# casselineau/Tracer

Measured on AMD Instinct MI355X. Metric: Mray-bounces/s on Sandia NSTTF field, higher is better.
Workload: dtype f64

## Files before the change

### tracer_amd/csrc/trc_bounds.h

```cpp
#ifndef TRC_BOUNDS_H
#define TRC_BOUNDS_H

#include <cmath>
#include <cstdlib>
#include <cstring>
#include <limits>
#include <vector>
#include "trc_core.h"

static inline bool trc_surface_local_box(const trc_surface_desc &s, double l[3], double h[3], bool *global_axes) {
    const double *g = s.gm;
    *global_axes = false;
    switch (s.gm_kind) {
    case TRC_GM_RECT: case TRC_GM_RECT_EXTRUDED: case TRC_GM_RECT_PERFORATED:
        l[0] = -g[0]; h[0] = g[0]; l[1] = -g[1]; h[1] = g[1]; l[2] = h[2] = 0.0; break;
    case TRC_GM_ROUND: case TRC_GM_ROUND_CUT:
        l[0] = l[1] = -g[0]; h[0] = h[1] = g[0]; l[2] = h[2] = 0.0; break;
    case TRC_GM_TRIANGLE:
        for (int i = 0; i < 3; ++i) { l[i] = std::fmin(0.0, std::fmin(g[i], g[3 + i])); h[i] = std::fmax(0.0, std::fmax(g[i], g[3 + i])); }
        break;
    case TRC_GM_POLYGON:
        l[0] = g[2]; h[0] = g[3]; l[1] = g[4]; h[1] = g[5]; l[2] = h[2] = 0.0; break;
    case TRC_GM_PARAB_DISH: {
        double rx = std::sqrt(g[2] / g[0]), ry = std::sqrt(g[2] / g[1]);
        l[0] = -rx; h[0] = rx; l[1] = -ry; h[1] = ry; l[2] = 0.0; h[2] = g[2]; break;
// ... 195 lines not shown
}

struct trc_accel_host {
    std::vector<float> sbox;
    std::vector<float> obb;
    std::vector<int32_t> unbounded;
    std::vector<uint32_t> nodes;
    std::vector<uint16_t> leaf_surfs;
    std::vector<uint16_t> brute_leaf;
    uint32_t brute_nodes[2];
    float brute_root[6];
    float root[6];
    float delta;
    double cen[3], slo[3], shi[3];
    bool any_bounded;
    int kd_depth;
    bool grid_ok;
    int32_t grid_dim[3];
    float grid_lo[3], grid_cs[3], grid_inv[3];
    std::vector<uint16_t> grid_off;
    std::vector<uint16_t> grid_list;
    std::vector<int32_t> grid_apart;
    float grid_root[6];
    bool big_ok;
    std::vector<int32_t> big_apart;
    int32_t big_dim[3];
    float big_lo[3], big_cs[3], big_inv[3], big_root[6];
    std::vector<uint32_t> big_off, big_list;
    std::vector<float> big_ent;
    std::vector<uint32_t> big_occ;
};

static inline void trc_accel_build_surfaces(const trc_surface_desc *surfs, int n, trc_accel_host &A) {
    const double INF = std::numeric_limits<double>::infinity();
    std::vector<double> lo(3 * (size_t)n), hi(3 * (size_t)n);
    std::vector<char> bounded(n);
    double slo[3] = {INF, INF, INF}, shi[3] = {-INF, -INF, -INF};
    A.unbounded.clear();
    A.any_bounded = false;
    for (int i = 0; i < n; ++i) {
        bounded[i] = trc_surface_bounds(surfs[i], &lo[3 * (size_t)i], &hi[3 * (size_t)i]);
        if (bounded[i]) {
            A.any_bounded = true;
            for (int k = 0; k < 3; ++k) { slo[k] = std::fmin(slo[k], lo[3 * (size_t)i + k]); shi[k] = std::fmax(shi[k], hi[3 * (size_t)i + k]); }
        } else A.unbounded.push_back(i);
    }
// ... 136 lines not shown
                range[6 * j + k] = a; range[6 * j + 3 + k] = z;
                c *= (size_t)(z - a + 1);
            }
            total += c;
        }
        if (total > 65535) continue;
        for (size_t j = 0; j < nb; ++j)
            for (int z = range[6 * j + 2]; z <= range[6 * j + 5]; ++z)
                for (int y = range[6 * j + 1]; y <= range[6 * j + 4]; ++y)
                    for (int x = range[6 * j]; x <= range[6 * j + 3]; ++x) count[((size_t)z * dim[1] + y) * dim[0] + x + 1]++;
        for (size_t c = 0; c < cells; ++c) count[c + 1] += count[c];
        A.grid_off.assign(cells + 1, 0);
        for (size_t c = 0; c <= cells; ++c) A.grid_off[c] = (uint16_t)count[c];
        A.grid_list.assign(total > 0 ? total : 1, 0);
        std::vector<uint32_t> cur(count.begin(), count.end() - 1);
        for (size_t j = 0; j < nb; ++j)
            for (int z = range[6 * j + 2]; z <= range[6 * j + 5]; ++z)
                for (int y = range[6 * j + 1]; y <= range[6 * j + 4]; ++y)
                    for (int x = range[6 * j]; x <= range[6 * j + 3]; ++x)
                        A.grid_list[cur[((size_t)z * dim[1] + y) * dim[0] + x]++] = members[j];
        for (int k = 0; k < 3; ++k) { A.grid_dim[k] = dim[k]; A.grid_lo[k] = (float)lo[k]; A.grid_cs[k] = cs[k]; A.grid_inv[k] = inv[k]; }
        A.grid_ok = true;
        return;
    }
}

static inline bool trc_tri_box_overlap(const double c[3], const double h[3], const double v0[3], const double v1[3], const double v2[3]) {
    double a[3][3], e[3][3];
    for (int i = 0; i < 3; ++i) { a[0][i] = v0[i] - c[i]; a[1][i] = v1[i] - c[i]; a[2][i] = v2[i] - c[i]; }
    for (int i = 0; i < 3; ++i) { e[0][i] = a[1][i] - a[0][i]; e[1][i] = a[2][i] - a[1][i]; e[2][i] = a[0][i] - a[2][i]; }
    double scale = 0.0;
    for (int k = 0; k < 3; ++k) for (int i = 0; i < 3; ++i) scale = std::fmax(scale, std::fabs(a[k][i]));
    for (int i = 0; i < 3; ++i) scale = std::fmax(scale, h[i]);
    const double tol = 1e-12 * scale;
    for (int i = 0; i < 3; ++i) {
        const double mn = std::fmin(a[0][i], std::fmin(a[1][i], a[2][i])), mx = std::fmax(a[0][i], std::fmax(a[1][i], a[2][i]));
        if (mn > h[i] + tol || mx < -h[i] - tol) return false;
    }
    {
        const double n[3] = {e[0][1] * e[1][2] - e[0][2] * e[1][1], e[0][2] * e[1][0] - e[0][0] * e[1][2], e[0][0] * e[1][1] - e[0][1] * e[1][0]};
        const double d = n[0] * a[0][0] + n[1] * a[0][1] + n[2] * a[0][2];
        const double rr = h[0] * std::fabs(n[0]) + h[1] * std::fabs(n[1]) + h[2] * std::fabs(n[2]);
        if (std::fabs(d) > rr + tol * (std::fabs(n[0]) + std::fabs(n[1]) + std::fabs(n[2]))) return false;
    }
    for (int k = 0; k < 3; ++k)
        for (int i = 0; i < 3; ++i) {
// ... 247 lines not shown
```

### tracer_amd/csrc/trc_core.h

```cpp
#ifndef TRC_CORE_H
#define TRC_CORE_H

#include <stdint.h>
#include <math.h>
#include "../../include/tracer_amd.h"

#if defined(__HIPCC__)
#define TRC_HD __host__ __device__ __forceinline__
#define TRC_HD_NOINLINE __host__ __device__
#else
#define TRC_HD static inline
#define TRC_HD_NOINLINE static
#endif

#define TRC_INF (__builtin_inf())
#define TRC_INF32 (__builtin_inff())
#define TRC_NAN (__builtin_nan(""))
#define TRC_TWO_PI 6.283185307179586476925286766559
#define TRC_PI 3.14159265358979323846264338327950288
#define TRC_BUIE_TABLE (3 * (TRC_BUIE_NELEM + 1) + 6)
#define TRC_BUIE_STAGED (TRC_BUIE_TABLE + 3)

#define TRC_REC_HDR 14

// ... 585 lines not shown
    float ax = (b[0] - r.ox) * r.ix, bx = (b[3] - r.ox) * r.ix;
    float ay = (b[1] - r.oy) * r.iy, by = (b[4] - r.oy) * r.iy;
    float az = (b[2] - r.oz) * r.iz, bz = (b[5] - r.oz) * r.iz;
    float lo = fmaxf(fmaxf(fminf(ax, bx), fminf(ay, by)), fmaxf(fminf(az, bz), 0.0f));
    float hi = fminf(fminf(fmaxf(ax, bx), fmaxf(ay, by)), fmaxf(az, bz));
    return hi * 1.0001f + 1e-6f >= lo;
}

TRC_HD bool trc_obb_hit32(const float *B, float ox, float oy, float oz, float dx, float dy, float dz) {
    const float rx = ox - B[3], ry = oy - B[7], rz = oz - B[11];
    const float lx = B[0] * rx + B[1] * ry + B[2] * rz, ly = B[4] * rx + B[5] * ry + B[6] * rz, lz = B[8] * rx + B[9] * ry + B[10] * rz;
    const float ex = B[0] * dx + B[1] * dy + B[2] * dz, ey = B[4] * dx + B[5] * dy + B[6] * dz, ez = B[8] * dx + B[9] * dy + B[10] * dz;
#if defined(__HIP_DEVICE_COMPILE__)
    const float ix = __builtin_amdgcn_rcpf(ex), iy = __builtin_amdgcn_rcpf(ey), iz = __builtin_amdgcn_rcpf(ez);
#else
    const float ix = 1.0f / ex, iy = 1.0f / ey, iz = 1.0f / ez;
#endif
    const float ax = (B[12] - lx) * ix, bx = (B[15] - lx) * ix;
    const float ay = (B[13] - ly) * iy, by = (B[16] - ly) * iy;
    const float az = (B[14] - lz) * iz, bz = (B[17] - lz) * iz;
    const float lo = fmaxf(fmaxf(fminf(ax, bx), fminf(ay, by)), fmaxf(fminf(az, bz), 0.0f));
    const float hi = fminf(fminf(fmaxf(ax, bx), fmaxf(ay, by)), fmaxf(az, bz));
    return hi * 1.0001f + 1e-6f >= lo;
}

TRC_HD bool trc_tri_hit32(float v0x, float v0y, float v0z, float e1x, float e1y, float e1z, float E, float e2x, float e2y, float e2z,
                          float emax2, float delta, const trc_ray32 &r) {
    const float tx = r.ox - v0x, ty = r.oy - v0y, tz = r.oz - v0z;
    const float px = fmaf(r.dy, e2z, -(r.dz * e2y)), py = fmaf(r.dz, e2x, -(r.dx * e2z)), pz = fmaf(r.dx, e2y, -(r.dy * e2x));
    const float det = fmaf(e1x, px, fmaf(e1y, py, e1z * pz));
    const float qx = fmaf(ty, e1z, -(tz * e1y)), qy = fmaf(tz, e1x, -(tx * e1z)), qz = fmaf(tx, e1y, -(ty * e1x));
    float u = fmaf(tx, px, fmaf(ty, py, tz * pz));
    float v = fmaf(r.dx, qx, fmaf(r.dy, qy, r.dz * qz));
    float tn = fmaf(e2x, qx, fmaf(e2y, qy, e2z * qz));
    if (det < 0.0f) { u = -u; v = -v; tn = -tn; }
    const float ad = fabsf(det);
    if (!(ad > 1e-5f * emax2)) return true;
    return u >= -E && v >= -E && u + v <= ad + 2.0f * E && tn >= -delta * (ad + emax2);
}

TRC_HD uint32_t trc_kd32_step(uint32_t w0, uint32_t w1, const trc_ray32 &r, float delta, float tmin, float *tmax,
                              bool *push, uint32_t *push_na, float *push_t) {
    uint32_t axis = w1 & 3u;
    float split = __builtin_bit_cast(float, w0);
    float o = axis == 0 ? r.ox : (axis == 1 ? r.oy : r.oz);
    float iv = axis == 0 ? r.ix : (axis == 1 ? r.iy : r.iz);
// ... 1418 lines not shown
```

### tracer_amd/csrc/trc_device.h

```cpp
#ifndef TRC_DEVICE_H
#define TRC_DEVICE_H

#include <hip/hip_runtime.h>
#include "trc_core.h"
#include "trc_bounds.h"
#include "trc_footprint.h"
#include "trc_forms.h"

struct FluxMapDev {
    int32_t surf, nu, nv, chart;
    int64_t edges_u, edges_v;
    int64_t bins;
    double proj[12];
};
static_assert(sizeof(FluxMapDev) == 136, "tests/shade_cases.py (SIZEOF_FLUXMAPDEV) restates this size in the sums of the LDS images");

struct DScene {
    const double *recs;
    const double *opt;
    const int32_t *sflags;
    const double *extra;
    int32_t stride, n_surf, n_extra, has_kd;
    const int32_t *kd_a, *kd_b, *kd_leaf, *kd_always;
    const double *kd_split;
// ... 399 lines not shown
    int static_general;
    FpDev fp;
    int static_first;
    int lds_recs;
    int lds_tables;
    int lds_fm_bins;
    int lds_extra;
    int bounce_no;
    int bg_occ_words;
    int split_terminal;
    unsigned chunk_thit;
    int search;
    int shade_cls;
    int shade_term_cls;
    long long act_base0;
    unsigned chunk_hitbuf;
    const uint32_t *hl_slot, *hl_surf;
    const double *hl_t;
    long long hl_room;
    int hl_cn;
    unsigned part_chunk[3];
    int part_static[3];
    CarryIn carry;
};

template <class ARGS>
__device__ __forceinline__ const ARGS *kernel_args_again() {
    static_assert(std::is_trivially_copyable<ARGS>::value, "the block is read as the bytes the launch copied into the segment");
    auto p = __builtin_amdgcn_kernarg_segment_ptr();
    asm volatile("" : "+s"(p));
    return (const ARGS *)p;
}

#define TRC_SURF_CLS_SHIFT 17
#define TRC_SURF_CLS_MASK 0x3
template <int THREADS>
__device__ __forceinline__ int wg_next(int i) {
    if constexpr (THREADS > 0) return i + THREADS;
    else return i + blockDim.x;
}

__device__ __forceinline__ void nearest_linked(const SCand *q3n, uint32_t k, double &t, int &s) {
    while (k != SQ_INVALID) {
        const SCand c = q3n[k];
        if (c.t < t || (c.t == t && (int)c.surf < s)) { t = c.t; s = (int)c.surf; }
        k = c.next;
// ... 255 lines not shown
```

### tracer_amd/csrc/trc_forms.h

```cpp
#ifndef TRC_FORMS_H
#define TRC_FORMS_H

#include <cstdio>
#include "trc_bounds.h"
#include "trc_footprint.h"

#define SC_THREADS 512
#define SC_GEN_CAP 1024
#define SF_THREADS(FLAT) ((FLAT) ? 1024 : 768)
#define SF2_DERIVES_CELL(FLAT, LDS) ((FLAT) || (LDS))
#ifndef SW_LEAFCAP
#define SW_LEAFCAP 16
#endif
#ifndef SW_LIST_T
#define SW_LIST_T uint16_t
#endif
#ifndef SW_THREADS
#define SW_THREADS 256
#endif
#define SB_THREADS 1024
#define SB_THREADS_OF(GRIDM) (SB_THREADS)
#define SA_THREADS 1024
#ifndef SHC_THREADS
#define SHC_THREADS 1024
// ... 76 lines not shown
    p.tables = p.sbox = lds;
    p.flags = flags;
    if (grid_cells) { p.grid_cells = grid_cells; p.grid_list = grid_list; }
    p.coop_waves = coop_waves;
    return p;
}
static inline size_t lds_need(const trc_lds_layout &L) { return L.end + L.slack; }
static inline size_t lds_request(const trc_lds_layout &L) { return lds_need(L) + 16; }
static inline size_t shade_lds_need(const trc_shade_parts &p) { const trc_shade_layout L = trc_shade_lds_layout(p); return L.end + L.slack; }

struct StreamKnobs {
    int search;
    bool fresh;
    bool bounce;
    bool first;
    bool coop;
    int absorb;
    bool static_chunks;
    bool room_set; long long room;
    long long q3_entries;
    int fp_cells;
    bool umask;
    int slots;
};

struct trc_scene_facts {
    int n_surf, stride;
    bool accel_ok, accel_kd_ok, has_kd;
    int kd_nodes, kd_nleaf, kd_nalways, kd_depth;
    bool grid_ok, big_ok;
    int grid_cells, grid_list;
    int brute_list, n_unbounded;
    int big_occ_words;
    int n_fm_edges, fms_bytes, n_extra;
    long long fm_bins;
    bool chart;
    bool transfer;
    bool splits;
    bool walked;
    bool all_flat;
    bool simple;
    unsigned cls_moving, cls_all;
    bool any_term;
};
struct trc_call_facts {
    long long n;
// ... 430 lines not shown
```

### tracer_amd/csrc/trc_kernels.hip

```cpp

#include <algorithm>
#include <cmath>
#include <cstdarg>
#include <cstdio>
#include <cstdlib>
#include <cstring>
#include <memory>
#include <mutex>
#include <new>
#include <string>
#include <unordered_map>
#include <utility>
#include <vector>

#include <hip/hip_runtime.h>
#include <rocprim/rocprim.hpp>

#include "trc_core.h"
#include "trc_bounds.h"
#include "trc_footprint.h"
#include "trc_device.h"
#include "trc_pool.h"
#include "trc_scene_host.h"
#include "trc_hithist.h"
// ... 264 lines not shown
    DevBuf<int32_t> d_sflags_;
public:
    int create(const trc_surface_desc *surfs, int32_t n, int32_t n_extra, const double *extra);
    int upload();
    void set_frames(const double *frames12) {
        for (size_t i = 0; i < surfs_.size(); ++i) memcpy(surfs_[i].frame, frames12 + 12 * i, 12 * sizeof(double));
    }
    const std::vector<trc_surface_desc> &all() const { return surfs_; }
    const trc_surface_desc *data() const { return surfs_.data(); }
    const trc_surface_desc &operator[](int i) const { return surfs_[i]; }
    bool splits() const { return splits_; }
    const CarryNeeds &needs() const { return needs_; }
    void fill(DScene &d) const {
        d.recs = d_recs_.get(); d.opt = d_opt_.get(); d.sflags = d_sflags_.get(); d.extra = d_extra_.get();
        d.stride = stride_; d.n_surf = (int32_t)surfs_.size(); d.n_extra = n_extra_;
    }
    void facts(trc_scene_facts &s) const { s.stride = stride_; s.n_extra = n_extra_; s.splits = splits_; }
};

class SearchTables {
    trc_accel_host accel_{};
    bool ok_ = false, kd_ok_ = false;
    uint64_t geom_version_ = 0;
    DevBuf<float> d_sbox_, d_obb_, d_bg_ent_;
    DevBuf<uint32_t> d_nodes_, d_bg_off_, d_bg_occ_;
    DevBuf<uint16_t> d_leaf_, d_bleaf_, d_goff_, d_glist_;
    DevBuf<int32_t> d_unbounded_, d_gapart_, d_bg_apart_;
    int build(const trc_surface_desc *surfs, int n);
public:
    int rebuild(const trc_surface_desc *surfs, int n) {
        const uint64_t version = geom_version_ + 1;
        SearchTables t;
        const int st = t.build(surfs, n);
        *this = st == TRC_OK ? std::move(t) : SearchTables();
        geom_version_ = version;
        return st;
    }
    int pack_kd(const trc_kdtree_desc *kd) {
        drop_kd();
        if (!ok_ || !trc_accel_build_kd(kd, accel_)) return TRC_OK;
        DevBuf<uint32_t> nodes;
        DevBuf<uint16_t> leaf;
        TRC_TRY(dev_upload(nodes, accel_.nodes.data(), accel_.nodes.size()));
        TRC_TRY(dev_upload(leaf, accel_.leaf_surfs.data(), accel_.leaf_surfs.size()));
        d_nodes_ = std::move(nodes); d_leaf_ = std::move(leaf);
        kd_ok_ = true;
        return TRC_OK;
    }
    void drop_kd() { d_nodes_.reset(); d_leaf_.reset(); kd_ok_ = false; }
    const trc_accel_host &host() const { return accel_; }
    uint64_t geom_version() const { return geom_version_; }
    void fill(DScene &d) const;
    void facts(trc_scene_facts &s) const { s.accel_ok = ok_; s.accel_kd_ok = kd_ok_; }
};

int SearchTables::build(const trc_surface_desc *surfs, int n) {
    const char *ev = getenv("TRC_GRID_FORCE32");
    trc_accel_host &A = accel_;
    trc_search_tables_build(surfs, n, ev && atoi(ev), A);
    TRC_TRY(dev_upload(d_obb_, A.obb.data(), A.obb.size()));
    TRC_TRY(dev_upload(d_bleaf_, A.brute_leaf.data(), A.brute_leaf.size()));
    TRC_TRY(dev_upload(d_sbox_, A.sbox.data(), A.sbox.size()));
    TRC_TRY(dev_upload(d_unbounded_, A.unbounded.data(), A.unbounded.size()));
    if (A.grid_ok) {
        TRC_TRY(dev_upload(d_gapart_, A.grid_apart.data(), A.grid_apart.size()));
        TRC_TRY(dev_upload(d_goff_, A.grid_off.data(), A.grid_off.size()));
        TRC_TRY(dev_upload(d_glist_, A.grid_list.data(), A.grid_list.size()));
    } else if (A.big_ok) {
        TRC_TRY(dev_upload(d_bg_off_, A.big_off.data(), A.big_off.size()));
        TRC_TRY(dev_upload(d_bg_ent_, A.big_ent.data(), A.big_ent.size()));
        TRC_TRY(dev_upload(d_bg_occ_, A.big_occ.data(), A.big_occ.size()));
        std::vector<float>().swap(A.big_ent);
        TRC_TRY(d_bg_apart_.alloc(A.big_apart.size() + 1));
        if (!A.big_apart.empty())
            HIP_TRY(hipMemcpy(d_bg_apart_.get(), A.big_apart.data(), A.big_apart.size() * sizeof(int32_t), hipMemcpyHostToDevice));
    }
    ok_ = true;
    return TRC_OK;
}

void SearchTables::fill(DScene &d) const {
    if (!ok_) return;
    const trc_accel_host &A = accel_;
    d.a_sbox = d_sbox_.get(); d.a_obb = d_obb_.get(); d.a_nodes = d_nodes_.get(); d.a_leaf = d_leaf_.get(); d.a_unbounded = d_unbounded_.get();
    d.a_n_unbounded = (int32_t)A.unbounded.size(); d.a_kd_depth = A.kd_depth;
    d.a_bleaf = d_bleaf_.get(); d.a_n_bleaf = (int32_t)A.brute_leaf.size();
    d.a_bnodes[0] = A.brute_nodes[0]; d.a_bnodes[1] = A.brute_nodes[1];
    d.a_ok = 1; d.a_kd_ok = kd_ok_ ? 1 : 0;
    d.a_delta = A.delta;
    d.a_goff = d_goff_.get(); d.a_glist = d_glist_.get(); d.a_gapart = d_gapart_.get();
// ... 2831 lines not shown
```

### tracer_amd/csrc/trc_scene_host.h

```cpp
#ifndef TRC_SCENE_HOST_H
#define TRC_SCENE_HOST_H

#include <algorithm>
#include <cstdarg>
#include <cstdio>
#include <vector>
#include "trc_bounds.h"

struct CarryNeeds {
    int max_mat = -1;
    bool poly = false;
    bool any() const { return max_mat >= 0 || poly; }
};

static inline int trc_refuse(char *msg, size_t len, int code, const char *fmt, ...) {
    va_list ap;
    va_start(ap, fmt);
    vsnprintf(msg, len, fmt, ap);
    va_end(ap);
    return code;
}

static inline int trc_surface_check(const trc_surface_desc &s, int idx, int n_extra, char *msg, size_t len) {
#define TRC_REFUSE(code, ...) return trc_refuse(msg, len, code, __VA_ARGS__)
// ... 49 lines not shown
    }
    int32_t *h = (int32_t *)(rec + 12);
    h[0] = s.gm_kind; h[1] = s.optics_kind; h[2] = s.extra_off; h[3] = s.extra_len;
    int np = trc_gm_nparams(s.gm_kind);
    for (int i = 0; i < np; ++i) rec[TRC_REC_HDR + i] = s.gm[i];
}

static inline void trc_scene_scan(const trc_surface_desc *surfs, int n, bool *splits, CarryNeeds *needs) {
    *splits = false;
    *needs = CarryNeeds();
    for (int i = 0; i < n; ++i) {
        const trc_surface_desc &s = surfs[i];
        if (s.optics_kind == TRC_OPT_REFRACTIVE_HOMOGENOUS && s.opt[2] == 0.0) *splits = true;
        if (s.optics_kind == TRC_OPT_REFRACTIVE_MATERIAL && s.opt[0] == 0.0) *splits = true;
        if (s.optics_kind == TRC_OPT_REFRACTIVE_MATERIAL) needs->max_mat = std::max(needs->max_mat, std::max((int)s.opt[4], (int)s.opt[5]));
        if (s.optics_kind == TRC_OPT_LAMBERTIAN_POLYCHROMATIC) needs->poly = true;
    }
}

static inline void trc_search_tables_build(const trc_surface_desc *surfs, int n, bool force32, trc_accel_host &A) {
    trc_accel_build_surfaces(surfs, n, A);
    trc_accel_build_grid(A, n);
    if (force32) A.grid_ok = false;
    if (!A.grid_ok) trc_accel_build_grid32(surfs, n, A);
}

#define TRC_KD_MAX_COUNT (1 << 29)
static inline int trc_kd_check(const trc_kdtree_desc *kd, int n_surf, int *max_depth_out, char *msg, size_t len) {
    *max_depth_out = 0;
    if (kd->n_nodes <= 0 || kd->n_leaf_surfs < 0 || kd->n_always < 0) TRC_REFUSE(TRC_ERR_INVALID, "incomplete tree (%d nodes, %d leaf entries, %d always relevant)", kd->n_nodes, kd->n_leaf_surfs, kd->n_always);
    if (kd->n_nodes >= TRC_KD_MAX_COUNT || kd->n_leaf_surfs >= TRC_KD_MAX_COUNT || kd->n_always >= TRC_KD_MAX_COUNT) TRC_REFUSE(TRC_ERR_INVALID, "tree too large");
    if (!kd->flag || !kd->split || !kd->child || !kd->leaf_off || !kd->leaf_cnt || (kd->n_leaf_surfs > 0 && !kd->leaf_surfs) ||
        (kd->n_always > 0 && !kd->always_relevant)) TRC_REFUSE(TRC_ERR_INVALID, "incomplete tree (an array is missing)");
    std::vector<int32_t> depth((size_t)kd->n_nodes, 0);
    for (int i = 0; i < kd->n_nodes; ++i) {
        const int f = kd->flag[i];
        if (f < 0 || f > 3) TRC_REFUSE(TRC_ERR_INVALID, "node %d: flag %d", i, f);
        if (f == 3) {
            const int64_t off = kd->leaf_off[i], cnt = kd->leaf_cnt[i];
            if (off < 0 || cnt < 0 || off + cnt > (int64_t)kd->n_leaf_surfs) TRC_REFUSE(TRC_ERR_INVALID, "node %d: leaf range", i);
        } else {
            const int64_t c = kd->child[i];
            if (c <= i || c + 1 >= (int64_t)kd->n_nodes) TRC_REFUSE(TRC_ERR_INVALID, "node %d: child %d out of range", i, (int)c);
            depth[c] = depth[c + 1] = depth[i] + 1;
            if (depth[c] > *max_depth_out) *max_depth_out = depth[c];
        }
// ... 37 lines not shown
```

### tracer_amd/csrc/trc_stream.inc

```


template <bool FRESH, int KIND>
__device__ __forceinline__ void s_gen_body(const StreamParams &S, trc_buie_fast &l_bf) {
    const FastParams &P = S.P;
    const DScene &sc = P.sc;
    const StreamWs &W = S.W;
    const bool buie_src = FRESH && P.src && (P.src->kind == TRC_SRC_BUIE_DISK || P.src->kind == TRC_SRC_BUIE_RECT);
    if (buie_src) trc_buie_fast_fill(P.src->buie, &l_bf, 0, (int)threadIdx.x, (int)blockDim.x);
    __syncthreads();
    if (buie_src) trc_buie_fast_fill(P.src->buie, &l_bf, 1, (int)threadIdx.x, (int)blockDim.x);
    __syncthreads();
    const trc_accel_view A = stream_accel_global(sc, S.search);
    const uint32_t *list = FRESH ? S.gen_list : S.act_in;
    long long count = FRESH ? (list ? (long long)W.cnt[CN(CW_GEN_LIST)] : S.nb) : (long long)W.cnt[CN(CW_ACT_IN)];
    if (list && count > (FRESH ? SQ_ROOM(W) : W.act_room)) count = FRESH ? SQ_ROOM(W) : W.act_room;
    const long long padded = (count + 63) & ~63ll;
    const unsigned long long wave_g = ((unsigned long long)blockIdx.x * blockDim.x + threadIdx.x) >> 6;
    WaveChunk c1 = S.static_general ? chunk_init_static(S.chunk_q1, wave_g) : chunk_init(S.chunk_q1);
    WaveChunk c3 = (!FRESH && S.q3_gen_chunk0 >= 0) ? chunk_init_static(S.chunk_q3, (unsigned long long)S.q3_gen_chunk0 + wave_g) : chunk_init(S.chunk_q3);
    WaveChunk cs = (FRESH && S.static_general) ? chunk_init_static_at(SQ_CHUNK, (unsigned long long)S.slot_base0 + wave_g * SQ_CHUNK) : chunk_init();
    for (long long i = (long long)blockIdx.x * blockDim.x + threadIdx.x; i < padded; i += (long long)gridDim.x * blockDim.x) {
        bool valid = i < count;
        uint32_t slot = 0, ri = 0;
        double px = 0, py = 0, pz = 0, dx = 0, dy = 0, dz = 1, e = 0, ref = 1.0, wl = 0.0;
// ... 814 lines not shown
            if (valid) in = trc_ray32_prepare(A.slo, A.shi, A.cen, px, py, pz, dx, dy, dz, &r, &t0);
            for (int s = 0; s < Sn; ++s) {
                const float *b = sc.a_sbox + 6 * (size_t)s;
                const bool unbounded = b[3] == TRC_INF && b[0] == -TRC_INF;
                bool cand = valid && s != skip;
                if (cand && !unbounded)
                    cand = in && trc_box_hit32(b, r) && trc_obb_hit32(sc.a_obb + (size_t)TRC_OBB_STRIDE * s, r.ox, r.oy, r.oz, r.dx, r.dy, r.dz);
                if (__ballot(cand)) {
                    if (cand) SB_TEST(s);
                }
            }
        } else
        if (valid) {
            for (int k = 0; k < A.n_unbounded; ++k) SB_PUSH(A.unbounded[k]);
            in = trc_ray32_prepare(A.slo, A.shi, A.cen, px, py, pz, dx, dy, dz, &r, &t0);
            if (in) {
                for (int k = 0; k < A.n_always; ++k) {
                    const int sidx = A.always[k];
                    const float *b = A.sbox + 6 * (size_t)sidx;
                    if (b[3] == TRC_INF && b[0] == -TRC_INF) continue;
                    if (trc_box_hit32(b, r) && trc_obb_hit32(obb + (size_t)(LDS ? TRC_OBB_LSTRIDE : TRC_OBB_STRIDE) * sidx, r.ox, r.oy, r.oz, r.dx, r.dy, r.dz)) SB_PUSH(sidx);
                }
                walk = trc_kd32_root(A.root, r, &tmin, &tmax);
            }
        }
        SB_FLUSH();
        if (GRID) {
            trc_dda dd;
            dd.cx = dd.cy = dd.cz = 0; dd.tnx = dd.tny = dd.tnz = 0.0f;
            if (walk) trc_dda_start(G, r, tmin, &dd);
            float t_enter = tmin;
            if (GRIDM == 2) {
                const float4 *ent = (const float4 *)sc.a_bg_ent;
                unsigned kc = 0, kc1 = 0;
                float4 n0 = make_float4(0.0f, 0.0f, 0.0f, 0.0f), n1 = n0, n2 = n0;
                while (__ballot(walk || kc < kc1)) {
                    if (lane_id() == 0) SB_COUNT(5, 1);
                    if (kc < kc1) {
                        SB_COUNT(1, 1);
                        const float4 c0 = n0, c1 = n1, c2 = n2;
                        ++kc;
                        if (kc < kc1) { n0 = ent[3 * (size_t)kc]; n1 = ent[3 * (size_t)kc + 1]; n2 = ent[3 * (size_t)kc + 2]; }
                        const uint32_t w = __float_as_uint(c0.x);
                        const int sidx = (int)(w & 0x7FFFFFFFu);
                        if (sidx != skip) {
                            bool pass;
// ... 817 lines not shown
        q3_cap = want;
        return TRC_OK;
    }
};

#define STREAM_MAX_SLOTS 4
static StreamKnobs stream_knobs() {
    StreamKnobs K;
    const char *ev;
    K.search = (ev = getenv("TRC_STREAM_SEARCH")) ? atoi(ev) : 2;
    K.fresh = !((ev = getenv("TRC_STREAM_FRESH")) && !atoi(ev));
    K.bounce = !((ev = getenv("TRC_STREAM_BOUNCE")) && !atoi(ev));
    K.first = (ev = getenv("TRC_STREAM_FIRST")) && atoi(ev);
    K.coop = !((ev = getenv("TRC_STREAM_COOP")) && !atoi(ev));
    K.absorb = (ev = getenv("TRC_STREAM_ABSORB")) ? atoi(ev) : -1;
    K.static_chunks = !((ev = getenv("TRC_STREAM_STATIC")) && !atoi(ev));
    K.room_set = (ev = getenv("TRC_STREAM_ROOM")) != nullptr;
    K.room = K.room_set && atoll(ev) >= 64 ? atoll(ev) : 0;
    K.q3_entries = (ev = getenv("TRC_STREAM_Q3_ENTRIES")) && atoll(ev) > 0 ? atoll(ev) : 0;
    K.fp_cells = (ev = getenv("TRC_STREAM_FP_CELLS")) && atoi(ev) >= 32 ? atoi(ev) : 0;
    K.umask = !((ev = getenv("TRC_STREAM_UMASK")) && !atoi(ev));
    K.slots = (ev = getenv("TRC_STREAM_SLOTS")) ? atoi(ev) : 2;
    if (K.slots < 1 || K.slots > STREAM_MAX_SLOTS) K.slots = 2;
    return K;
}

#define STREAM_ACT_STATIC(cap) ((cap) + ((cap) >> 2) + (1ll << 23))

static int stream_ws_alloc_queues(StreamBuffers &W, long long cap, long long want_q3, long long want_room, const StreamKnobs &K) {
    const size_t cq = (size_t)want_room;
    const long long act_room = K.room ? want_room
                             : 2 * STREAM_ACT_STATIC(cap) + cap + (1ll << 20);
    TRC_TRY(W.geo.alloc(cq));
    TRC_TRY(W.aux.alloc(cq));
    TRC_TRY(W.q1_slot.alloc(cq));
    TRC_TRY(W.q1_a.alloc(cq));
    TRC_TRY(W.q1_b.alloc(cq));
    TRC_TRY(W.q3_slot.alloc((size_t)want_q3));
    TRC_TRY(W.q3_surf.alloc((size_t)want_q3));
    TRC_TRY(W.q3n.alloc((size_t)want_q3));
    TRC_TRY(W.hit_slot.alloc(cq));
    TRC_TRY(W.hit_surf.alloc(cq));
    TRC_TRY(W.hit_t.alloc(cq));
    TRC_TRY(W.gen_list.alloc(cq));
    TRC_TRY(W.fq_ray.alloc(cq));
    TRC_TRY(W.fq_cell.alloc(cq));
// ... 253 lines not shown
        trc_kernel_name(s.id, name, sizeof(name));
        return trc_fail(TRC_ERR_UNSUPPORTED, "the library holds no kernel %s", name);
    }
    if (cap) TRC_TRY(kernel_grid_cap(k.fn, k.threads, lds_cap, 2048 / k.threads, n_cu, &k.max_blocks));
    return (cap && lds_cap == k.lds) ? TRC_OK : kernel_allow_lds(k.fn, k.lds);
}

static int stream_choose_forms(StreamForms &F, StreamParams &SP0, trc_scene *sc, StreamEngine &E, const StreamPlan &plan, trc_facts &f,
                               const trc_source_desc *src_desc) {
    const int n_cu = sc->ctx->n_cu;
    memset(&F, 0, sizeof(F));
    f.scene = scene_facts(sc, true);
    f.fp = {};
    TRC_TRY(stream_fp_prepare(sc, E, src_desc, f.knobs, &SP0.fp, &f.fp.use));
    if (f.fp.use) {
        const trc_fp_host &H = *E.fp;
        f.fp = {true, SP0.fp.n_list, H.P.M, H.P.Mc, H.P.has_generic != 0, H.P.cdf_end, H.coverage, H.ucoverage, E.d_fp_umask.get() ? (int)H.umask.size() : 0, H.Mu, H.Mv};
    }
    trc_stream_forms &D = F.D;
    if (!trc_stream_decide(f, plan, &D)) return trc_fail(TRC_ERR_UNSUPPORTED, "no shading kernel for device material tables beside a chart flux map");
    SP0.search = D.search; SP0.lds_recs = D.lds_recs; SP0.P.lds_tally = D.lds_tally; SP0.lds_tables = D.lds_tables; SP0.lds_extra = D.lds_extra;
    SP0.lds_fm_bins = D.lds_fm_bins; SP0.bg_occ_words = D.bg_occ_words; SP0.shade_term_cls = D.shade_term_cls; SP0.split_terminal = D.split_terminal;
    SP0.carry.poly_cells = D.poly_cells;
    SP0.hit_epoch = sc->hits.epoch;
    SP0.chunk_hitbuf = sc->hits.chunk_size();
    TRC_TRY(stream_stage(F.gen0, D.gen0, n_cu, false, 0));
    TRC_TRY(stream_stage(F.gen, D.gen, n_cu, false, 0));
    TRC_TRY(stream_stage(F.walk, D.walk, n_cu, true, D.walk.lds));
    TRC_TRY(stream_stage(F.exact, D.exact, n_cu, false, 0));
    F.g_wide = (unsigned)(n_cu * 8);
    F.g_gen = (unsigned)(n_cu * 8);
    for (int q = 0; q < D.n_shk; ++q) {
        const trc_shade_stage &s = D.shk[q];
        StreamKernel k;
        const bool cap = s.id.family != TRC_K_SHADE;
        TRC_TRY(stream_stage(k, {s.id, s.threads, s.lds}, n_cu, cap, s.lds));
        StreamShadeK &K = F.shk[q];
        K = {s.cls, k.fn, (unsigned)s.threads, (unsigned)s.threads / 64, cap ? k.max_blocks : (unsigned)(n_cu * 4), s.lds, s.lds_tables, s.lds_fm_bins};
        if (cap && (unsigned long long)K.max_blocks * K.wpb > SHADE_MAX_WAVES) K.max_blocks = SHADE_MAX_WAVES / K.wpb;
    }
    TRC_TRY(stream_stage(F.cull, D.cull, n_cu, true, D.cull.lds));
    TRC_TRY(stream_stage(F.fresh, D.fresh, n_cu, true, D.fresh.lds));
    if (trc_kid_equal(D.fresh_one.id, D.fresh.id)) F.fresh_one = {F.fresh.fn, F.fresh.threads, F.fresh.lds, 0u};
    else TRC_TRY(stream_stage(F.fresh_one, D.fresh_one, n_cu, false, 0));
    TRC_TRY(stream_stage(F.cull_u, D.cull_u, n_cu, true, D.cull_u.lds));
    if (F.cull_u.fn) {
// ... 489 lines not shown
    if (rc != TRC_OK) {
        for (int k = 0; k < n_slots; ++k)
            if (E.slot[k].W.tally_part) (void)hipMemset(E.slot[k].W.tally_part.get(), 0, (size_t)TALLY_PARTS * (size_t)E.slot[k].W.tally_n * sizeof(double));
        return rc;
    }
    HIP_TRY(hipEventRecord(ctx->ev1, ctx->stream));
    HIP_TRY(hipStreamSynchronize(ctx->stream));
    float total_ms = 0;
    (void)hipEventElapsedTime(&total_ms, ctx->ev0, ctx->ev1);
    for (int k = 0; k < n_slots; ++k)
        hipLaunchKernelGGL(k_s_merge_tallies, dim3((unsigned)((sc->tally.size() + 255) / 256)), dim3(256), 0, ctx->stream, sc->tally.device(), E.slot[k].W.tally_part.get(), (long long)sc->tally.size());
    hipLaunchKernelGGL(k_s_add2, dim3(1), dim3(64), 0, ctx->stream, sc->tally.device() + 3 * sc->n_surf, C.seg, C.hits);
    stats->kernel_ms = total_ms;
#ifdef SB_STATS
    {
        unsigned long long h[32];
        if (hipMemcpyFromSymbol(h, HIP_SYMBOL(g_sb_stats), sizeof(h)) == hipSuccess) {
            for (int f = 0; f < 2; ++f) {
                const unsigned long long *q = h + 16 * f;
                const double nr = q[7] ? (double)q[7] : 1.0, nw = q[9] ? (double)q[9] : 1.0;
                fprintf(stderr, "k_s_bounce, %s rays: %llu in %llu wave passes; per ray: cells %.2f (occupied %.2f), entries %.2f, passed %.2f, exact tests %.2f; "
                                "per wave pass: walk turns %.1f, rounds of exact tests %.1f\n", f ? "continued" : "fresh", q[7], q[9], q[0] / nr, q[4] / nr, q[1] / nr,
                        q[2] / nr, q[3] / nr, q[5] / nw, q[6] / nw);
            }
            memset(h, 0, sizeof(h));
            hipMemcpyToSymbol(HIP_SYMBOL(g_sb_stats), h, sizeof(h));
        }
    }
#endif
    stats->launches = C.launches + 1;
    stats->bounces = C.max_bounces;
    *seg_out = C.seg;
    *hit_out = C.hits;
    return TRC_OK;
}
```

Baseline: 69830.

## Skip grid walk for reflected rays inside precomputed per-heliostat clear cones

Precomputes on the host, for each flat facet (heliostat) and each tile of an 8x8 tiling, a cone around the direction to the receiver that no other surface can occlude. In the bounce kernel, continued rays leaving such a facet whose direction falls inside the tile's cone skip the acceleration-structure walk entirely and go straight to the receiver (apart) tests. This removes most of the grid traversal for reflected rays in a heliostat field, at the cost of an extra host-side build step, a small table lookup per ray, and correctness risk if the conservative cone bounds are wrong.

```diff
diff --git a/tracer_amd/csrc/trc_bounds.h b/tracer_amd/csrc/trc_bounds.h
--- a/tracer_amd/csrc/trc_bounds.h
+++ b/tracer_amd/csrc/trc_bounds.h
@@ -1,6 +1,7 @@
 #ifndef TRC_BOUNDS_H
 #define TRC_BOUNDS_H
 
+#include <algorithm>
 #include <cmath>
 #include <cstdlib>
 #include <cstring>
@@ -242,6 +243,8 @@
     std::vector<uint16_t> grid_list;
     std::vector<int32_t> grid_apart;
     float grid_root[6];
+    std::vector<float> clear;
+    int32_t clear_T = 0, clear_cones = 0;
     bool big_ok;
     std::vector<int32_t> big_apart;
     int32_t big_dim[3];
@@ -424,6 +427,193 @@
         for (int k = 0; k < 3; ++k) { A.grid_dim[k] = dim[k]; A.grid_lo[k] = (float)lo[k]; A.grid_cs[k] = cs[k]; A.grid_inv[k] = inv[k]; }
         A.grid_ok = true;
         return;
+    }
+}
+
+#define TRC_CLEAR_CAP 0.2
+
+struct trc_clear_box { double c[8][3]; double cen[3], rad; };
+
+static inline void trc_clear_box_finish(trc_clear_box &b) {
+    for (int i = 0; i < 3; ++i) { b.cen[i] = 0.0; for (int c = 0; c < 8; ++c) b.cen[i] += 0.125 * b.c[c][i]; }
+    b.rad = 0.0;
+    for (int c = 0; c < 8; ++c) {
+        double r2 = 0.0;
+        for (int i = 0; i < 3; ++i) r2 += (b.c[c][i] - b.cen[i]) * (b.c[c][i] - b.cen[i]);
+        b.rad = std::fmax(b.rad, std::sqrt(r2));
+    }
+}
+static inline void trc_clear_box_of(const float *B, const double l[3], const double h[3], trc_clear_box &b) {
+    for (int c = 0; c < 8; ++c) {
+        const double p[3] = {(c & 1) ? h[0] : l[0], (c & 2) ? h[1] : l[1], (c & 4) ? h[2] : l[2]};
+        for (int i = 0; i < 3; ++i) b.c[c][i] = (double)B[4 * i + 3] + (double)B[i] * p[0] + (double)B[4 + i] * p[1] + (double)B[8 + i] * p[2];
+    }
+    trc_clear_box_finish(b);
+}
+static inline double trc_clear_tan(const trc_clear_box &P, const trc_clear_box &Q, const double a[3], const double e1[3], const double e2[3],
+                                   double bound, bool *exact) {
+    double p2[8][2], q2[8][2], pmin = INFINITY, qmax = -INFINITY;
+    *exact = true;
+    for (int c = 0; c < 8; ++c) {
+        pmin = std::fmin(pmin, a[0] * P.c[c][0] + a[1] * P.c[c][1] + a[2] * P.c[c][2]);
+        qmax = std::fmax(qmax, a[0] * Q.c[c][0] + a[1] * Q.c[c][1] + a[2] * Q.c[c][2]);
+        for (int k = 0; k < 2; ++k) {
+            const double *e = k ? e2 : e1;
+            p2[c][k] = e[0] * P.c[c][0] + e[1] * P.c[c][1] + e[2] * P.c[c][2];
+            q2[c][k] = e[0] * Q.c[c][0] + e[1] * Q.c[c][1] + e[2] * Q.c[c][2];
+        }
+    }
+    const double smax = qmax - pmin;
+    if (!(smax > 0.0)) return INFINITY;
+    double gap = 0.0;
+    for (int w = 0; w < 2; ++w)
+        for (int bit = 1; bit < 8; bit <<= 1) {
+            const double (*z)[2] = w ? q2 : p2;
+            const double nx = -(z[bit][1] - z[0][1]), ny = z[bit][0] - z[0][0], nn = nx * nx + ny * ny;
+            if (!(nn > 0.0)) continue;
+            double p0 = INFINITY, p1 = -INFINITY, q0 = INFINITY, q1 = -INFINITY;
+            for (int c = 0; c < 8; ++c) {
+                const double pp = nx * p2[c][0] + ny * p2[c][1], qq = nx * q2[c][0] + ny * q2[c][1];
+                p0 = std::fmin(p0, pp); p1 = std::fmax(p1, pp); q0 = std::fmin(q0, qq); q1 = std::fmax(q1, qq);
+            }
+            const double g = std::fmax(q0 - p1, p0 - q1);
+            if (g > 0.0) gap = std::fmax(gap, g / std::sqrt(nn));
+        }
+    if (!(gap > 0.0)) return 0.0;
+    if (gap * (1.0 - 1e-12) / smax >= bound) { *exact = false; return gap * (1.0 - 1e-12) / smax; }
+    double d2 = INFINITY;
+    for (int w = 0; w < 2; ++w) {
+        const double (*z)[2] = w ? q2 : p2, (*o)[2] = w ? p2 : q2;
+        for (int c = 0; c < 8; ++c)
+            for (int bit = 1; bit < 8; bit <<= 1) {
+                if (c & bit) continue;
+                const double ex = z[c | bit][0] - z[c][0], ey = z[c | bit][1] - z[c][1], ee = ex * ex + ey * ey, ie = ee > 0.0 ? 1.0 / ee : 0.0;
+                for (int v = 0; v < 8; ++v) {
+                    const double wx = o[v][0] - z[c][0], wy = o[v][1] - z[c][1];
+                    double t = (wx * ex + wy * ey) * ie;
+                    t = t < 0.0 ? 0.0 : (t > 1.0 ? 1.0 : t);
+                    const double rx = wx - t * ex, ry = wy - t * ey;
+                    d2 = std::fmin(d2, rx * rx + ry * ry);
+                }
+            }
+    }
+    return std::sqrt(d2) * (1.0 - 1e-12) / smax;
+}
+
+static inline void trc_clear_build(const trc_surface_desc *surfs, int n_surf, int T, trc_accel_host &A) {
+    A.clear.clear();
+    A.clear_T = T;
+    A.clear_cones = 0;
+    if (!A.grid_ok || A.grid_apart.empty() || T < 1) return;
+    A.clear.assign((size_t)n_surf * T * T * 4, 0.0f);
+    const double delta = (double)A.delta, tcap = std::tan(TRC_CLEAR_CAP);
+    std::vector<char> listed((size_t)n_surf, 0);
+    for (size_t k = 0; k < (size_t)A.grid_off.back() && k < A.grid_list.size(); ++k) listed[A.grid_list[k]] = 1;
+    std::vector<int> ids;
+    std::vector<trc_clear_box> boxes;
+    for (int g = 0; g < n_surf; ++g) {
+        if (!listed[g]) continue;
+        const float *B = &A.obb[(size_t)TRC_OBB_STRIDE * g];
+        const double l[3] = {B[12], B[13], B[14]}, h[3] = {B[15], B[16], B[17]};
+        trc_clear_box b;
+        trc_clear_box_of(B, l, h, b);
+        ids.push_back(g);
+        boxes.push_back(b);
+    }
+    double target[3] = {0.0, 0.0, 0.0};
+    for (int32_t s : A.grid_apart) {
+        const float *B = &A.obb[(size_t)TRC_OBB_STRIDE * s];
+        const double l[3] = {B[12], B[13], B[14]}, h[3] = {B[15], B[16], B[17]};
+        trc_clear_box b;
+        trc_clear_box_of(B, l, h, b);
+        for (int i = 0; i < 3; ++i) target[i] += b.cen[i] / (double)A.grid_apart.size();
+    }
+    std::vector<int> near, keep;
+    std::vector<std::vector<int>> lists, below;
+    for (size_t hi = 0; hi < ids.size(); ++hi) {
+        const int hs = ids[hi];
+        const int kind = surfs[hs].gm_kind;
+        const float *B = &A.obb[(size_t)TRC_OBB_STRIDE * hs];
+        if (!trc_gm_is_flat(kind) || kind == TRC_GM_TRIANGLE || !(B[14] < 0.0f && B[17] > 0.0f && B[14] == -B[17])) continue;
+        const trc_clear_box &H = boxes[hi];
+        double a[3] = {target[0] - H.cen[0], target[1] - H.cen[1], target[2] - H.cen[2]};
+        const double an = std::sqrt(a[0] * a[0] + a[1] * a[1] + a[2] * a[2]);
+        if (!(an > 0.0)) continue;
+        for (int i = 0; i < 3; ++i) a[i] /= an;
+        const float af[3] = {(float)a[0], (float)a[1], (float)a[2]};
+        const double fn = std::sqrt((double)af[0] * af[0] + (double)af[1] * af[1] + (double)af[2] * af[2]);
+        for (int i = 0; i < 3; ++i) a[i] = (double)af[i] / fn;
+        const int m = std::fabs(a[0]) < std::fabs(a[1]) ? (std::fabs(a[0]) < std::fabs(a[2]) ? 0 : 2) : (std::fabs(a[1]) < std::fabs(a[2]) ? 1 : 2);
+        double e1[3] = {0.0, 0.0, 0.0}, e2[3];
+        e1[m] = 1.0;
+        const double d1 = a[m];
+        double n1 = 0.0;
+        for (int i = 0; i < 3; ++i) { e1[i] -= d1 * a[i]; n1 += e1[i] * e1[i]; }
+        n1 = std::sqrt(n1);
+        for (int i = 0; i < 3; ++i) e1[i] /= n1;
+        e2[0] = a[1] * e1[2] - a[2] * e1[1]; e2[1] = a[2] * e1[0] - a[0] * e1[2]; e2[2] = a[0] * e1[1] - a[1] * e1[0];
+        auto outside = [&](const trc_clear_box &P, const trc_clear_box &Q, double t) {
+            const double v[3] = {Q.cen[0] - P.cen[0], Q.cen[1] - P.cen[1], Q.cen[2] - P.cen[2]};
+            const double s = a[0] * v[0] + a[1] * v[1] + a[2] * v[2], R = P.rad + Q.rad;
+            if (s + R <= 0.0) return true;
+            const double w2 = v[0] * v[0] + v[1] * v[1] + v[2] * v[2] - s * s, reach = t * (s + R) + R;
+            return w2 >= reach * reach;
+        };
+        near.clear();
+        for (size_t gi = 0; gi < ids.size(); ++gi) if (gi != hi && !outside(H, boxes[gi], tcap)) near.push_back((int)gi);
+        std::sort(near.begin(), near.end(), [&](int x, int y) {
+            const double sx = a[0] * boxes[(size_t)x].cen[0] + a[1] * boxes[(size_t)x].cen[1] + a[2] * boxes[(size_t)x].cen[2];
+            const double sy = a[0] * boxes[(size_t)y].cen[0] + a[1] * boxes[(size_t)y].cen[1] + a[2] * boxes[(size_t)y].cen[2];
+            return sx < sy || (sx == sy && x < y);
+        });
+        const double lo[2] = {B[12], B[13]}, up[2] = {B[15], B[16]};
+        lists.assign(1, near);
+        for (int L = (T & (T - 1)) ? T : 1; L <= T; L *= 2) {
+            const bool last = L == T;
+            if (!last) below.assign((size_t)4 * L * L, std::vector<int>());
+            for (int tv = 0; tv < L; ++tv)
+                for (int tu = 0; tu < L; ++tu) {
+                    const std::vector<int> &list = lists[lists.size() == 1 ? 0 : (size_t)tv * L + tu];
+                    const int t2[2] = {tu, tv};
+                    double l[3], h[3];
+                    for (int k = 0; k < 2; ++k) {
+                        const double w = (up[k] - lo[k]) / L;
+                        l[k] = std::fmax(lo[k], lo[k] + t2[k] * w - 2.0 * delta);
+                        h[k] = std::fmin(up[k], lo[k] + (t2[k] + 1) * w + 2.0 * delta);
+                    }
+                    l[2] = B[14]; h[2] = B[17];
+                    trc_clear_box P;
+                    trc_clear_box_of(B, l, h, P);
+                    double tmin = tcap;
+                    keep.clear();
+                    for (size_t j = 0; j < list.size(); ++j) {
+                        if (!(tmin > 0.0)) {
+                            if (last) break;
+                            keep.push_back(list[j]);
+                            continue;
+                        }
+                        const trc_clear_box &Q = boxes[(size_t)list[j]];
+                        if (outside(P, Q, tcap)) continue;
+                        if (tmin < tcap && outside(P, Q, tmin)) { keep.push_back(list[j]); continue; }
+                        bool exact;
+                        const double t = trc_clear_tan(P, Q, a, e1, e2, tmin, &exact);
+                        if (t >= tcap) continue;
+                        keep.push_back(list[j]);
+                        if (exact) tmin = std::fmin(tmin, t);
+                    }
+                    if (!last) {
+                        for (int c = 0; c < 4; ++c) below[(size_t)(2 * tv + (c >> 1)) * (2 * L) + (2 * tu + (c & 1))] = keep;
+                        continue;
+                    }
+                    const double alpha = std::fmax(std::atan(tmin) * (1.0 - 1e-3) - 1e-4, 0.0), tk = std::tan(alpha);
+                    float k = trc_f32_down(tk * tk);
+                    if (!(k > 0.0f)) k = 0.0f;
+                    float *o = &A.clear[((size_t)hs * T * T + (size_t)tv * T + tu) * 4];
+                    o[0] = af[0]; o[1] = af[1]; o[2] = af[2]; o[3] = k;
+                    if (k > 0.0f) A.clear_cones += 1;
+                }
+            if (!last) lists.swap(below);
+        }
     }
 }
 
diff --git a/tracer_amd/csrc/trc_core.h b/tracer_amd/csrc/trc_core.h
--- a/tracer_amd/csrc/trc_core.h
+++ b/tracer_amd/csrc/trc_core.h
@@ -631,6 +631,27 @@
     const float lo = fmaxf(fmaxf(fminf(ax, bx), fminf(ay, by)), fmaxf(fminf(az, bz), 0.0f));
     const float hi = fminf(fminf(fmaxf(ax, bx), fmaxf(ay, by)), fmaxf(az, bz));
     return hi * 1.0001f + 1e-6f >= lo;
+}
+
+#ifndef TRC_CLEAR_T
+#define TRC_CLEAR_T 8
+#endif
+TRC_HD int trc_clear_tile(const float *B, int T, float ox, float oy, float oz) {
+    const float rx = ox - B[3], ry = oy - B[7], rz = oz - B[11];
+    const float lu = B[0] * rx + B[1] * ry + B[2] * rz, lv = B[4] * rx + B[5] * ry + B[6] * rz;
+#if defined(__HIP_DEVICE_COMPILE__)
+    const float su = (float)T * __builtin_amdgcn_rcpf(B[15] - B[12]), sv = (float)T * __builtin_amdgcn_rcpf(B[16] - B[13]);
+#else
+    const float su = (float)T / (B[15] - B[12]), sv = (float)T / (B[16] - B[13]);
+#endif
+    const int tu = (int)fminf(fmaxf((lu - B[12]) * su, 0.0f), (float)(T - 1));
+    const int tv = (int)fminf(fmaxf((lv - B[13]) * sv, 0.0f), (float)(T - 1));
+    return tv * T + tu;
+}
+TRC_HD bool trc_clear_inside(float ax, float ay, float az, float k, float dx, float dy, float dz) {
+    const float c = dx * ax + dy * ay + dz * az;
+    const float xx = dy * az - dz * ay, xy = dz * ax - dx * az, xz = dx * ay - dy * ax;
+    return c > 0.0f && xx * xx + xy * xy + xz * xz < k * (c * c);
 }
 
 TRC_HD bool trc_tri_hit32(float v0x, float v0y, float v0z, float e1x, float e1y, float e1z, float E, float e2x, float e2y, float e2z,
diff --git a/tracer_amd/csrc/trc_device.h b/tracer_amd/csrc/trc_device.h
--- a/tracer_amd/csrc/trc_device.h
+++ b/tracer_amd/csrc/trc_device.h
@@ -445,6 +445,7 @@
     unsigned part_chunk[3];
     int part_static[3];
     CarryIn carry;
+    const float *clear_tab;
 };
 
 template <class ARGS>
diff --git a/tracer_amd/csrc/trc_forms.h b/tracer_amd/csrc/trc_forms.h
--- a/tracer_amd/csrc/trc_forms.h
+++ b/tracer_amd/csrc/trc_forms.h
@@ -122,6 +122,7 @@
     int fp_cells;
     bool umask;
     int slots;
+    bool clear = true;
 };
 
 struct trc_scene_facts {
diff --git a/tracer_amd/csrc/trc_kernels.hip b/tracer_amd/csrc/trc_kernels.hip
--- a/tracer_amd/csrc/trc_kernels.hip
+++ b/tracer_amd/csrc/trc_kernels.hip
@@ -310,7 +310,7 @@
     trc_accel_host accel_{};
     bool ok_ = false, kd_ok_ = false;
     uint64_t geom_version_ = 0;
-    DevBuf<float> d_sbox_, d_obb_, d_bg_ent_;
+    DevBuf<float> d_sbox_, d_obb_, d_bg_ent_, d_clear_;
     DevBuf<uint32_t> d_nodes_, d_bg_off_, d_bg_occ_;
     DevBuf<uint16_t> d_leaf_, d_bleaf_, d_goff_, d_glist_;
     DevBuf<int32_t> d_unbounded_, d_gapart_, d_bg_apart_;
@@ -338,6 +338,7 @@
     void drop_kd() { d_nodes_.reset(); d_leaf_.reset(); kd_ok_ = false; }
     const trc_accel_host &host() const { return accel_; }
     uint64_t geom_version() const { return geom_version_; }
+    const float *clear_cones() const { return ok_ && accel_.clear_cones > 0 ? d_clear_.get() : nullptr; }
     void fill(DScene &d) const;
     void facts(trc_scene_facts &s) const { s.accel_ok = ok_; s.accel_kd_ok = kd_ok_; }
 };
@@ -354,6 +355,7 @@
         TRC_TRY(dev_upload(d_gapart_, A.grid_apart.data(), A.grid_apart.size()));
         TRC_TRY(dev_upload(d_goff_, A.grid_off.data(), A.grid_off.size()));
         TRC_TRY(dev_upload(d_glist_, A.grid_list.data(), A.grid_list.size()));
+        if (A.clear_cones > 0) TRC_TRY(dev_upload(d_clear_, A.clear.data(), A.clear.size()));
     } else if (A.big_ok) {
         TRC_TRY(dev_upload(d_bg_off_, A.big_off.data(), A.big_off.size()));
         TRC_TRY(dev_upload(d_bg_ent_, A.big_ent.data(), A.big_ent.size()));
diff --git a/tracer_amd/csrc/trc_scene_host.h b/tracer_amd/csrc/trc_scene_host.h
--- a/tracer_amd/csrc/trc_scene_host.h
+++ b/tracer_amd/csrc/trc_scene_host.h
@@ -95,6 +95,7 @@
     trc_accel_build_surfaces(surfs, n, A);
     trc_accel_build_grid(A, n);
     if (force32) A.grid_ok = false;
+    trc_clear_build(surfs, n, TRC_CLEAR_T, A);
     if (!A.grid_ok) trc_accel_build_grid32(surfs, n, A);
 }
 
diff --git a/tracer_amd/csrc/trc_stream.inc b/tracer_amd/csrc/trc_stream.inc
--- a/tracer_amd/csrc/trc_stream.inc
+++ b/tracer_amd/csrc/trc_stream.inc
@@ -860,6 +860,13 @@
                     if (trc_box_hit32(b, r) && trc_obb_hit32(obb + (size_t)(LDS ? TRC_OBB_LSTRIDE : TRC_OBB_STRIDE) * sidx, r.ox, r.oy, r.oz, r.dx, r.dy, r.dz)) SB_PUSH(sidx);
                 }
                 walk = trc_kd32_root(A.root, r, &tmin, &tmax);
+                if constexpr (GRIDM == 1 && !FRESH) {
+                    if (walk && skip >= 0 && S.clear_tab && t0 == 0.0) {
+                        const int tile = trc_clear_tile(obb + (size_t)(LDS ? TRC_OBB_LSTRIDE : TRC_OBB_STRIDE) * skip, TRC_CLEAR_T, r.ox, r.oy, r.oz);
+                        const float4 cone = ((const float4 *)S.clear_tab)[(size_t)skip * (TRC_CLEAR_T * TRC_CLEAR_T) + tile];
+                        if (trc_clear_inside(cone.x, cone.y, cone.z, cone.w, r.dx, r.dy, r.dz)) { walk = false; SB_COUNT(10, 1); }
+                    }
+                }
             }
         }
         SB_FLUSH();
@@ -1723,6 +1730,7 @@
     K.umask = !((ev = getenv("TRC_STREAM_UMASK")) && !atoi(ev));
     K.slots = (ev = getenv("TRC_STREAM_SLOTS")) ? atoi(ev) : 2;
     if (K.slots < 1 || K.slots > STREAM_MAX_SLOTS) K.slots = 2;
+    K.clear = !((ev = getenv("TRC_STREAM_CLEAR")) && !atoi(ev));
     return K;
 }
 
@@ -2022,6 +2030,7 @@
     SP0.search = D.search; SP0.lds_recs = D.lds_recs; SP0.P.lds_tally = D.lds_tally; SP0.lds_tables = D.lds_tables; SP0.lds_extra = D.lds_extra;
     SP0.lds_fm_bins = D.lds_fm_bins; SP0.bg_occ_words = D.bg_occ_words; SP0.shade_term_cls = D.shade_term_cls; SP0.split_terminal = D.split_terminal;
     SP0.carry.poly_cells = D.poly_cells;
+    SP0.clear_tab = f.knobs.clear ? sc->search.clear_cones() : nullptr;
     SP0.hit_epoch = sc->hits.epoch;
     SP0.chunk_hitbuf = sc->hits.chunk_size();
     TRC_TRY(stream_stage(F.gen0, D.gen0, n_cu, false, 0));
@@ -2557,6 +2566,7 @@
                 fprintf(stderr, "k_s_bounce, %s rays: %llu in %llu wave passes; per ray: cells %.2f (occupied %.2f), entries %.2f, passed %.2f, exact tests %.2f; "
                                 "per wave pass: walk turns %.1f, rounds of exact tests %.1f\n", f ? "continued" : "fresh", q[7], q[9], q[0] / nr, q[4] / nr, q[1] / nr,
                         q[2] / nr, q[3] / nr, q[5] / nw, q[6] / nw);
+                if (f) fprintf(stderr, "k_s_bounce, continued rays inside a clear cone (no walk): %llu\n", q[10]);
             }
             memset(h, 0, sizeof(h));
             hipMemcpyToSymbol(HIP_SYMBOL(g_sb_stats), h, sizeof(h));
```

Measured after the change: 74680 (median of 6 runs). 1.07x the previous value.
